# cxjyxxme/deep-online-video-stabilization

Hardware: AMD Instinct MI355X
Metric: stabilized frames/sec (720p, before_ch=31) (higher is better)
Workload: dtype f32 (bf16x3 split MFMA, f32 accumulate); 1 GPU; BASELINE.json configs[1]: v2_93 net, 1280x720, 1 stream(s)/GPU, batch=1 per stream, 13-ch stack from a 32-deep ring (lags 1,2,4,8,16,32; --before-ch 31 ignored as in the reference), ResNet-v2-50 regressor + 4x4 multi-grid warp + feedback; one independent stream set per GPU (replicas only); height=720, width=1280, streams_per_gpu=1, refine=1, operand_mode=4, launches_per_frame=64, hip_graph=True

## Files before the change

deep-online-video-stabilization_amd/csrc/conv.hip:

```cpp
#include "conv.h"
#include "prof.h"
#include <climits>
#include <cstdio>
#include <cstdlib>
#include <algorithm>
#include <string>
#include <vector>

#include "conv_kernel.h"
#include "conv_ring_kernel.h"
#include "conv_astat_kernel.h"
#include "conv_patch_kernel.h"
#include "conv_b2b_kernel.h"

template <int PAIR>
__device__ __forceinline__ void conv_splitk_reduce_body(const ConvArgs& p, const ConvPair& pr) {
    const size_t q = (size_t)blockIdx.x * 256 + threadIdx.x;
    const int c4n = p.Cout / 4;
    if (q >= (size_t)p.M * c4n) return;
    const int m = (int)(q / c4n);
    const int n = (int)(q - (size_t)m * c4n) * 4;
    const bool t1 = PAIR && m >= pr.m_tower;
    const size_t slab = (size_t)p.M * p.Cout;
    const float* src = p.partial + (size_t)m * p.Cout + n;
// ... 428 lines not shown
    return r.nbuf == 1 ? launch_one_nb<BM, BN, BK, WM, WN, MODE, 1>(a, st) : launch_one_nb<BM, BN, BK, WM, WN, MODE, 2>(a, st);
}

template <int BM, int BN, int BK, int WM, int WN>
static int launch_one(const ConvRoute& r, const ConvArgs& a, hipStream_t st) {
    if (r.mode == 2) return launch_one_t<BM, BN, BK, WM, WN, 2>(r, a, st);
    if (r.mode == 0) return launch_one_t<BM, BN, BK, WM, WN, 0>(r, a, st);
    return launch_one_t<BM, BN, BK, WM, WN, 1>(r, a, st);
}

static int launch_igemm(const ConvRoute& r, const ConvArgs& a, hipStream_t st) {
    if (r.bk == 32) {
        if (r.tile == T128x128) return launch_one<128, 128, 32, 64, 64>(r, a, st);
        if (r.tile == T128x64) return launch_one<128, 64, 32, 64, 32>(r, a, st);
        return launch_one<64, 64, 32, 32, 32>(r, a, st);
    }
    if (r.tile == T128x128) return launch_one<128, 128, 16, 64, 64>(r, a, st);
    if (r.tile == T128x64) return launch_one<128, 64, 16, 64, 32>(r, a, st);
    return launch_one<64, 64, 16, 32, 32>(r, a, st);
}

static int device_cus(int& cus) {
    static int cached = 0;
    if (cached == 0) {
        int dev = 0, n = 0;
        if (hipGetDevice(&dev) != hipSuccess || hipDeviceGetAttribute(&n, hipDeviceAttributeMultiprocessorCount, dev) != hipSuccess || n <= 0) {
            stabnet_set_error("conv: cannot read the CU count");
            return STABNET_ERR_LAUNCH;
        }
        cached = n;
    }
    cus = cached;
    return STABNET_OK;
}
static thread_local int g_last_launch_kind = -1;

template <int B>
static bool launch_ring_operand(const ConvRoute& r, const ConvArgs& a, int grid, hipStream_t st) {
    const int key = 100 * r.mode + 10 * r.kg + r.pro;
    if (key == 10) { conv_ring_f32_kernel<0, B><<<grid, 256, 0, st>>>(a); return true; }
    if (key == 110) { conv_ring_f32_kernel<1, B><<<grid, 256, 0, st>>>(a); return true; }
    if (key == 210) { conv_ring_f32_kernel<2, B><<<grid, 256, 0, st>>>(a); return true; }
    if constexpr (B != 1) {
        if (key == 11) { conv_ring_f32_kernel<0, B, 1, 1><<<grid, 256, 0, st>>>(a); return true; }
        if (key == 21) { conv_ring_f32_kernel<0, B, 2, 1><<<grid, 512, 0, st>>>(a); return true; }
    }
    if constexpr (B == 0 || B == 2 || B == 3) {
        if (key == 30) { conv_ring_f32_kernel<0, B, 3><<<grid, 768, 0, st>>>(a); return true; }
        if (key == 130) { conv_ring_f32_kernel<1, B, 3><<<grid, 768, 0, st>>>(a); return true; }
    }
    if constexpr (B == 4) {
        if (key == 20) { conv_ring_f32_kernel<0, B, 2, 0><<<grid, 512, 0, st>>>(a); return true; }
        if (key == 120) { conv_ring_f32_kernel<1, B, 2, 0><<<grid, 512, 0, st>>>(a); return true; }
    }
    return false;
}

static int launch_ring_route(const ConvRoute& r, const ConvArgs& a, hipStream_t st) {
    int cus = 0;
    if (const int rc = device_cus(cus)) return rc;
    const int grid = ring_grid(r, a, cus).gx;
    bool ok = false;
    switch (r.operand) {
        case 0: ok = launch_ring_operand<0>(r, a, grid, st); break;
        case 1: ok = launch_ring_operand<1>(r, a, grid, st); break;
        case 2: ok = launch_ring_operand<2>(r, a, grid, st); break;
        case 3: ok = launch_ring_operand<3>(r, a, grid, st); break;
        case 4: ok = launch_ring_operand<4>(r, a, grid, st); break;
        default: break;
    }
    SN_REQUIRE(ok, "conv: no conv_ring_f32_kernel<%d, %d, %d, %d>", r.mode, r.operand, r.kg, r.pro);
    SN_LAUNCH_CHECK("conv_ring_f32_kernel");
    return STABNET_OK;
}

static int launch_astat(const ConvRoute& r, const ConvArgs& a, hipStream_t st) {
    int cus = 0;
    if (const int rc = device_cus(cus)) return rc;
    const int bm = r.astat_bm;
    SN_REQUIRE(bm == 32 && a.K % 32 == 0 && (size_t)bm * a.K * 6 <= (size_t)SN_ASTAT_A_BYTES && a.splitk == 1,
               "conv: the A-stationary kernel takes BM %d x K %d without a K split only if the planes fit %d bytes", bm, a.K, SN_ASTAT_A_BYTES);
    const ConvGrid g = astat_grid(a, bm, cus);
    const dim3 grid(g.gx, g.gy);
    conv_astat_f32_kernel<32><<<grid, 256, 0, st>>>(a);
    SN_LAUNCH_CHECK("conv_astat_f32_kernel");
    return STABNET_OK;
}

template <int PH, int PW, int WR, int NS>
static int launch_patch_one(const ConvArgs& a, int cus, hipStream_t st) {
    const size_t lds = sn_patch_lds_bytes(PH, PW, a.Cin);
    auto kern = conv_patch_f32_kernel<PH, PW, WR, NS>;
    static size_t configured = 64 * 1024;
    if (lds > configured) {
        hipError_t e = hipFuncSetAttribute(reinterpret_cast<const void*>(kern), hipFuncAttributeMaxDynamicSharedMemorySize, (int)SN_PATCH_LDS_MAX);
        if (e != hipSuccess) {
            stabnet_set_error("conv: hipFuncSetAttribute(%zu B LDS) failed: %s", SN_PATCH_LDS_MAX, hipGetErrorString(e));
            return STABNET_ERR_LAUNCH;
        }
        configured = SN_PATCH_LDS_MAX;
    }
    const ConvGrid g = patch_grid(a, PH, PW, WR, cus);
    const dim3 grid(g.gx, g.gy);
    kern<<<grid, 256, lds, st>>>(a);
    SN_LAUNCH_CHECK("conv_patch_f32_kernel");
    return STABNET_OK;
}
static int launch_patch(const ConvRoute& r, const ConvArgs& a, hipStream_t st) {
    int cus = 0;
    if (const int rc = device_cus(cus)) return rc;
    SN_REQUIRE(a.KH == 3 && a.KW == 3 && a.stride == 1 && a.pad == 1 && a.up == 1 && a.Cin % 32 == 0 &&
                   (a.splitk == 1 || (a.splitk == 2 && a.steps_per_split * 2 == conv_total_steps(a))) && a.Ho == a.H && a.Wo == a.W && r.patch_cfg >= 1 &&
                   r.patch_cfg <= SN_PATCH_FORMS &&
                   sn_patch_lds_bytes(g_patch_forms[r.patch_cfg - 1].ph, g_patch_forms[r.patch_cfg - 1].pw, a.Cin) <= SN_PATCH_LDS_MAX,
               "conv: the patch-stationary kernel takes 3x3 / pad 1 / stride 1 over Cin %d (a multiple of 32) without a K split or with two equal K halves only if the planes fit %zu bytes",
               a.Cin, SN_PATCH_LDS_MAX);
    return r.patch_cfg == 1 ? launch_patch_one<8, 8, 1, 3>(a, cus, st) : launch_patch_one<8, 8, 2, 3>(a, cus, st);
}

size_t conv_weight_image_floats(int Cout, int K) { return (size_t)cdiv(Cout, 64) * (size_t)(K / 32) * 3072; }

__device__ __forceinline__ unsigned weight_split_head(float& x0, float& x1) {
    const float top = __builtin_bit_cast(float, 0x7F7F0000u), fmax = __builtin_bit_cast(float, 0x7F7FFFFFu);
    const float h0 = (fabsf(x0) > top && fabsf(x0) <= fmax) ? copysignf(top, x0) : x0;
    const float h1 = (fabsf(x1) > top && fabsf(x1) <= fmax) ? copysignf(top, x1) : x1;
    const unsigned p = sn_pack_bf16(h0, h1);
    x0 = sn_sub_f32(x0, __builtin_bit_cast(float, p << 16));
    x1 = sn_sub_f32(x1, __builtin_bit_cast(float, p & 0xffff0000u));
    return p;
}
__device__ __forceinline__ SnSplit3 weight_split3(const f32x4 x) {
    float a = x.x, b = x.y, c = x.z, d = x.w;
    typedef unsigned u32x2 __attribute__((ext_vector_type(2)));
    u32x2 h, m, l;
    h.x = weight_split_head(a, b); h.y = weight_split_head(c, d);
    m.x = sn_split_level(a, b); m.y = sn_split_level(c, d);
    l.x = sn_pack_bf16(a, b); l.y = sn_pack_bf16(c, d);
    SnSplit3 s;
    s.h = __builtin_bit_cast(sn_bf16x4, h); s.m = __builtin_bit_cast(sn_bf16x4, m); s.l = __builtin_bit_cast(sn_bf16x4, l);
    return s;
}

__device__ __forceinline__ void weight_split_image_thread(const float* __restrict__ w, int Cout, int K, uint4* __restrict__ img, long i) {
    const int steps = K / 32;
    const int lane = (int)(i & 63), j = (int)((i >> 6) & 1), wn = (int)((i >> 7) & 1);
    const long ts = i >> 8;
    const int ks = (int)(ts % steps), nt = (int)(ts / steps);
    const int n = nt * 64 + wn * 32 + (lane & 31), g = lane >> 5;
    f32x4 lo = {0.f, 0.f, 0.f, 0.f}, hi = lo;
    if (n < Cout) {
        const float* r = w + (size_t)n * K + ks * 32 + 16 * j + 4 * g;
        lo = *reinterpret_cast<const f32x4*>(r);
        hi = *reinterpret_cast<const f32x4*>(r + 8);
    }
    const SnSplit3 a = weight_split3(lo), b = weight_split3(hi);
    uint4* out = img + ts * 768 + (size_t)(wn * 6 + j) * 64 + lane;
    out[0] = __builtin_bit_cast(uint4, SN_CAT8(a.h, b.h));
    out[2 * 64] = __builtin_bit_cast(uint4, SN_CAT8(a.m, b.m));
    out[4 * 64] = __builtin_bit_cast(uint4, SN_CAT8(a.l, b.l));
}

__global__ __launch_bounds__(256) void weight_split_image_kernel(const float* __restrict__ w, int Cout, int K, uint4* __restrict__ img) {
    const long i = (long)blockIdx.x * 256 + threadIdx.x;
    if (i >= (long)((Cout + 63) / 64) * (K / 32) * 256) return;
    weight_split_image_thread(w, Cout, K, img, i);
}

// ... 129 lines not shown
                       a.M, a.Cout, a.K, a.splitk);
    if (rc) return rc;
    if (a.splitk > 1) {
        const size_t q = (size_t)a.M * (a.Cout / 4);
        const bool rec2 = prof != nullptr && prof->begin(st);
        conv_splitk_reduce_pair_kernel<<<cdiv((long)q, 256), 256, 0, st>>>(a, pr);
        if (rec2) prof->end(st, PK_KERNEL_SPLITK_REDUCE, 0.0, 4.0 * (double)a.M * a.Cout * (a.splitk + 1));
        SN_LAUNCH_CHECK("conv_splitk_reduce_pair_kernel");
    }
    return STABNET_OK;
}

bool conv_b2b_supported(const ConvArgs& c2, const ConvArgs& c3) {
    const bool g2 = c2.KH == 3 && c2.KW == 3 && c2.pad == 1 && c2.up == 1 && !c2.rowrun && (c2.stride == 1 || c2.stride == 2) &&
                    c2.Cin == c2.Cout && (c2.Cout == 64 || c2.Cout == 128) && c2.in_scale_expected == 0 && c2.in_scale == nullptr;
    const bool g3 = c3.KH == 1 && c3.KW == 1 && c3.pad == 0 && c3.stride == 1 && c3.up == 1 && !c3.rowrun && c3.Cin == c2.Cout &&
                    (c3.x_ld == 0 || c3.x_ld == c3.Cin) && c3.Cout % c2.Cout == 0 && c3.N == c2.N && c3.H == c2.Ho && c3.W == c2.Wo &&
                    c3.in_scale_expected == 0 && c3.in_scale == nullptr;
    return sw().b2b && sw().ring && g2 && g3;
}

int conv_b2b_launch(const ConvArgs& c2, const ConvArgs& c3, hipStream_t st, Prof* prof) {
    SN_REQUIRE(conv_b2b_supported(c2, c3), "conv b2b: unsupported geometry");
    SN_REQUIRE(c2.div_hw_mul != 0 && c3.div_hw_mul != 0 && c2.M == c3.M, "conv b2b: conv_plan() not called on both convolutions");
    SN_REQUIRE(c2.x && c2.w && c3.w && c3.y && c2.out_scale && c2.out_shift, "conv b2b: null pointer");
    SN_REQUIRE(c2.bias == nullptr && c2.residual == nullptr, "conv b2b: the 3x3 convolution takes no bias / residual");
    int cus = 0;
    if (const int rc = device_cus(cus)) return rc;
    B2bArgs P;
    P.c2 = c2;
    P.c3 = c3;
    P.c3.splitk = 1;
    P.c3.steps_per_split = conv_total_steps(c3);
    const int tiles_m = cdiv(c2.M, 64);
    g_last_launch_kind = PK_KERNEL_CONV_B2B + (c2.Cout == 128 ? 1 : 0);
    const bool rec = prof != nullptr && prof->begin(st);
    if (c2.Cout == 64) {
        conv_b2b_f32_kernel<2><<<std::min(tiles_m, sw().b2b_wgs_per_cu * usable_cus(cus)), 256, 0, st>>>(P);
    } else {
        conv_b2b_f32_kernel<4><<<std::min(tiles_m, usable_cus(cus)), 512, 0, st>>>(P);
    }
    if (rec) prof->end(st, PK_KERNEL_CONV_B2B + (c2.Cout == 128 ? 1 : 0),
                       2.0 * c2.M * ((double)c2.K * c2.Cout + (double)c3.K * c3.Cout),
                       4.0 * ((double)c2.N * c2.H * c2.W * c2.Cin + (double)c2.K * c2.Cout + (double)c3.K * c3.Cout +
                              (double)c3.M * c3.Cout * (c3.residual ? 2 : 1)),
                       c2.M, c3.Cout, c2.K + c3.K, 1);
    SN_LAUNCH_CHECK("conv_b2b_f32_kernel");
    return STABNET_OK;
}

static int fill_args(ConvArgs& a, const float* x, const float* w, const float* bias, const float* in_scale,
                     const float* in_shift, const float* residual, int res_H, int res_W, int res_stride, float* y,
                     int N, int H, int W, int Cin, int Cout, int KH, int KW, int stride, int pad, int relu_out) {
    SN_REQUIRE(N > 0 && H > 0 && W > 0 && Cin > 0 && Cout > 0 && KH > 0 && KW > 0 && stride > 0 && pad >= 0,
               "conv2d: bad geometry");
    SN_REQUIRE(Cin % 16 == 0, "conv2d: Cin=%d must be a multiple of 16", Cin);
    SN_REQUIRE((in_scale == nullptr) == (in_shift == nullptr), "conv2d: in_scale and in_shift go together");
    a = ConvArgs{};
    a.x = x; a.w = w; a.y = y; a.bias = bias; a.in_scale = in_scale; a.in_shift = in_shift; a.residual = residual;
    a.in_scale_expected = in_scale != nullptr ? 1 : 0;
    a.N = N; a.H = H; a.W = W; a.Cin = Cin; a.Cout = Cout; a.KH = KH; a.KW = KW; a.stride = stride; a.pad = pad;
    a.up = 1;
    a.Ho = (H + 2 * pad - KH) / stride + 1;
    a.Wo = (W + 2 * pad - KW) / stride + 1;
    SN_REQUIRE(a.Ho > 0 && a.Wo > 0, "conv2d: empty output");
    a.res_H = residual ? res_H : a.Ho;
    a.res_W = residual ? res_W : a.Wo;
    a.res_stride = residual ? res_stride : 1;
    a.relu_out = relu_out;
    SN_REQUIRE((long)N * a.Ho * a.Wo * Cout < (1L << 30) && (long)N * (H + 2 * pad) * (W + 2 * pad) * Cin < (1L << 30) &&
                   (long)Cout * KH * KW * Cin < (1L << 30), "conv2d: tensors must have < 2^30 elements");
    SN_REQUIRE(KH * KW <= 64, "conv2d: filter larger than 64 taps");
    return STABNET_OK;
}

extern "C" {

int stabnet_conv_reserve_cus(int reserved) {
    const int prev = g_reserved_cus;
    g_reserved_cus = reserved < 0 ? 0 : reserved;
    return prev;
}

void stabnet_conv_tuning_override(int tile, int splitk) {
    g_force_tile = tile < 0 ? -1 : tile;
    g_force_split = splitk;
}

void stabnet_conv_tuning_profile(int profile) { g_tuning_profile = profile == 1 ? 1 : 0; }

void stabnet_conv_tuning_table_set(int M, int Cout, int K, int KH, int ring, int splitk) {
    if (M < 0) { g_tuning_runtime.clear(); return; }
    for (size_t i = 0; i < g_tuning_runtime.size(); ++i) {
        TuneEntry& e = g_tuning_runtime[i];
        if (e.M == M && e.Cout == Cout && e.K == K && e.KH == KH && e.ring == ring) {
            if (splitk > 0) e.splitk = splitk;
            else g_tuning_runtime.erase(g_tuning_runtime.begin() + i);
            return;
        }
    }
    if (splitk > 0) g_tuning_runtime.push_back({M, Cout, K, KH, ring, splitk});
}

size_t stabnet_conv2d_workspace_bytes(int N, int H, int W, int Cin, int Cout, int KH, int KW, int stride, int pad) {
    ConvArgs a;
    if (fill_args(a, nullptr, nullptr, nullptr, nullptr, nullptr, nullptr, 0, 0, 1, nullptr, N, H, W, Cin, Cout, KH, KW,
                  stride, pad, 0))
        return 0;
    ConvArgs b = a;
    b.in_scale_expected = 1;
    return std::max(conv_plan(a), conv_plan(b));
}

int stabnet_conv2d_fwd_ex(const float* x, const float* w_ohwi, const float* bias, const float* in_scale,
                          const float* in_shift, const float* residual, int res_H, int res_W, int res_stride,
                          const float* out_scale, const float* out_shift, float* y, int N, int H, int W, int Cin,
                          int Cout, int KH, int KW, int stride, int pad, int relu_out, void* workspace,
                          size_t workspace_bytes, void* stream);

int stabnet_conv2d_fwd(const float* x, const float* w_ohwi, const float* bias, const float* in_scale,
                       const float* in_shift, const float* residual, int res_H, int res_W, int res_stride, float* y,
                       int N, int H, int W, int Cin, int Cout, int KH, int KW, int stride, int pad, int relu_out,
                       void* workspace, size_t workspace_bytes, void* stream) {
    return stabnet_conv2d_fwd_ex(x, w_ohwi, bias, in_scale, in_shift, residual, res_H, res_W, res_stride, nullptr, nullptr,
                                 y, N, H, W, Cin, Cout, KH, KW, stride, pad, relu_out, workspace, workspace_bytes, stream);
}

int stabnet_conv_last_launch_kind(void) { return g_last_launch_kind; }

int stabnet_conv2d_fwd_ex(const float* x, const float* w_ohwi, const float* bias, const float* in_scale,
                          const float* in_shift, const float* residual, int res_H, int res_W, int res_stride,
                          const float* out_scale, const float* out_shift, float* y, int N, int H, int W, int Cin,
                          int Cout, int KH, int KW, int stride, int pad, int relu_out, void* workspace,
                          size_t workspace_bytes, void* stream) {
    SN_REQUIRE(x && w_ohwi && y, "conv2d_fwd: null pointer");
    SN_REQUIRE((out_scale == nullptr) == (out_shift == nullptr), "conv2d_fwd: out_scale and out_shift go together");
    ConvArgs a;
    int rc = fill_args(a, x, w_ohwi, bias, in_scale, in_shift, residual, res_H, res_W, res_stride, y, N, H, W, Cin, Cout,
                       KH, KW, stride, pad, relu_out);
    if (rc) return rc;
    const size_t need = conv_plan(a);
    if (need > workspace_bytes || (need > 0 && workspace == nullptr)) {
        stabnet_set_error("conv2d_fwd: workspace %zu B < %zu B needed", workspace_bytes, need);
        return STABNET_ERR_WORKSPACE;
    }
    a.partial = static_cast<float*>(workspace);
    a.out_scale = out_scale;
    a.out_shift = out_shift;
    return conv_launch(a, (hipStream_t)stream);
}

int stabnet_conv2d_fwd_packed_ld(const float* x, int x_ld, const float* w_ohwi, const float* w_img, const float* bias, const float* in_scale,
                                 const float* in_shift, const float* residual, int res_H, int res_W, int res_stride,
                                 const float* out_scale, const float* out_shift, float* y, int N, int H, int W, int Cin,
                                 int Cout, int KH, int KW, int stride, int pad, int relu_out, int splitk, void* workspace,
                                 size_t workspace_bytes, void* stream);
size_t stabnet_conv_weight_image_floats(int Cout, int KH, int KW, int Cin) {
    const int K = KH * KW * Cin;
    return (Cout > 0 && K > 0 && K % 32 == 0) ? conv_weight_image_floats(Cout, K) : 0;
}

int stabnet_conv_weight_split_image(const float* w_ohwi, int Cout, int KH, int KW, int Cin, float* w_img, void* stream) {
    SN_REQUIRE(w_ohwi && w_img, "conv_weight_split_image: null pointer");
    SN_REQUIRE(Cin % 32 == 0, "conv_weight_split_image: Cin=%d must be a multiple of 32", Cin);
    return launch_weight_split_image(w_ohwi, Cout, KH * KW * Cin, w_img, (hipStream_t)stream);
}
// ... 80 lines not shown
```

deep-online-video-stabilization_amd/csrc/conv_astat_kernel.h:

```cpp
#pragma once
#include "conv_kernel.h"

constexpr int SN_ASTAT_A_BYTES = 48 * 1024;

template <int BM>
__global__ __launch_bounds__(256, 2) void conv_astat_f32_kernel(const ConvArgs p) {
    static_assert(BM == 32 || BM == 64, "one or two 32-row blocks");
    constexpr int RB = BM / 32;
    typedef unsigned u32x2 __attribute__((ext_vector_type(2)));
    __shared__ __attribute__((aligned(16))) unsigned char lds[SN_ASTAT_A_BYTES + 4 * SN_EPI_WAVE_BYTES];

    const int tid = threadIdx.x, lane = tid & 63, wave = __builtin_amdgcn_readfirstlane(tid >> 6);
    const int steps = p.K >> 5, kq = 2 * steps;
    const ConvTile tile = conv_tile_of_block(p);
    const int m0 = tile.mt * BM, grp = tile.nt;

    {
        const int r = tid >> 3, sub = tid & 7;
        const unsigned ent = (unsigned)((r + 32 * (sub & 1)) * 16 + 8 * ((sub >> 1) & 1));
#pragma unroll
        for (int rb = 0; rb < RB; ++rb) {
            const int row = min(m0 + rb * 32 + r, p.M - 1);
            const float* src = p.x + (size_t)row * p.x_ld + sub * 4;
            for (int ks0 = 0; ks0 < steps; ks0 += 4) {
                f32x4 v[4];
#pragma unroll
                for (int i = 0; i < 4; ++i) v[i] = *reinterpret_cast<const f32x4*>(src + 32 * min(ks0 + i, steps - 1));
                __builtin_amdgcn_sched_barrier(0);
#pragma unroll
                for (int i = 0; i < 4; ++i) {
                    float a = v[i].x, b = v[i].y, c = v[i].z, d = v[i].w;
                    u32x2 h, m, l;
                    h.x = sn_split_level(a, b); h.y = sn_split_level(c, d);
                    m.x = sn_split_level(a, b); m.y = sn_split_level(c, d);
                    l.x = sn_pack_bf16(a, b); l.y = sn_pack_bf16(c, d);
                    unsigned char* dst = lds + (unsigned)((rb * kq + 2 * min(ks0 + i, steps - 1) + (sub >> 2)) * 3072) + ent;
                    *reinterpret_cast<u32x2*>(dst) = h;
                    *reinterpret_cast<u32x2*>(dst + 1024) = m;
                    *reinterpret_cast<u32x2*>(dst + 2048) = l;
                }
            }
        }
    }
    __syncthreads();

    const int nblk = 2 * ((p.Cout + 63) >> 6);
    const int bpg = (((nblk + (int)gridDim.y - 1) / (int)gridDim.y) + 3) & ~3;
    const int b_end = min(min(nblk, (grp + 1) * bpg), (p.Cout + 31) >> 5);
    int b = grp * bpg + wave;
    if (b >= b_end) return;
    const unsigned scratch = (unsigned)(size_t)(__attribute__((address_space(3))) void*)lds + (unsigned)(SN_ASTAT_A_BYTES + wave * SN_EPI_WAVE_BYTES);
    const f32x4* lp = reinterpret_cast<const f32x4*>(p.w) + ((size_t)(b >> 1) * steps * 12 + (b & 1) * 6) * 64 + lane;
    const unsigned char* afrag = lds + lane * 16;
    const int items = ((b_end - b + 3) >> 2) * steps;
    int l_item = 0, l_ks = 0;
    auto load = [&](f32x4 (&dst)[6]) {
#pragma unroll
        for (int i = 0; i < 6; ++i) dst[i] = lp[i * 64];
        const int adv = l_item + 1 >= items ? 0 : (l_ks + 1 < steps ? 768 : 768 * (steps + 1));
        lp += adv;
        ++l_item;
        l_ks = l_ks + 1 < steps ? l_ks + 1 : 0;
        __builtin_amdgcn_sched_barrier(0);
    };
    f32x16 acc[RB][1];
    auto zero = [&]() {
#pragma unroll
        for (int rb = 0; rb < RB; ++rb)
#pragma unroll
            for (int e = 0; e < 16; ++e) acc[rb][0][e] = 0.f;
    };
    int ks = 0;
    auto item = [&](const f32x4 (&B)[6]) {
#pragma unroll
        for (int j = 0; j < 2; ++j) {
#pragma unroll
            for (int rb = 0; rb < RB; ++rb) {
                const unsigned char* ap = afrag + (unsigned)((rb * kq + 2 * ks + j) * 3072);
                SnPlanes A;
                A.h = *reinterpret_cast<const sn_u32x4*>(ap);
                A.m = *reinterpret_cast<const sn_u32x4*>(ap + 1024);
                A.l = *reinterpret_cast<const sn_u32x4*>(ap + 2048);
                sn_mfma_split3_pk(acc[rb][0], A, B[j], B[2 + j], B[4 + j]);
            }
        }
        if (++ks == steps) {
            conv_epilogue<RB, 1>(acc, p, m0, b * 32, lane, 0, scratch);
            b += 4;
            ks = 0;
            zero();
        }
    };
    f32x4 B0[6], B1[6], B2[6];
    zero();
    load(B0);
    load(B1);
    for (int it = 0; it < items; it += 3) {
        load(B2); item(B0);
        if (it + 1 >= items) break;
        load(B0); item(B1);
        if (it + 2 >= items) break;
        load(B1); item(B2);
    }
}
```

deep-online-video-stabilization_amd/csrc/layers.hip:

```cpp
#include "layers.h"
#include <algorithm>

__global__ __launch_bounds__(256) void pad_channels_kernel(const float* __restrict__ x, float* __restrict__ y,
                                                           long npix, int C, int Cp) {
    const long q = (long)blockIdx.x * 256 + threadIdx.x;
    const int f4 = Cp / 4;
    if (q >= npix * f4) return;
    const long pix = q / f4;
    const int c = (int)(q - pix * f4) * 4;
    const float* s = x + pix * C;
    float4 v;
    v.x = (c + 0 < C) ? s[c + 0] : 0.f;
    v.y = (c + 1 < C) ? s[c + 1] : 0.f;
    v.z = (c + 2 < C) ? s[c + 2] : 0.f;
    v.w = (c + 3 < C) ? s[c + 3] : 0.f;
    *reinterpret_cast<float4*>(y + pix * Cp + c) = v;
}

__global__ __launch_bounds__(256) void max_pool_kernel(const float* __restrict__ x, float* __restrict__ y, int N, int H,
                                                       int W, int C, int Ho, int Wo, int k, int stride, int pt, int pl,
                                                       const float* __restrict__ scale, const float* __restrict__ shift) {
    const unsigned q = sn_xcd_band(blockIdx.x, gridDim.x) * 256u + threadIdx.x;
    const unsigned c4n = (unsigned)C / 4u;
    if (q >= (unsigned)N * Ho * Wo * c4n) return;
    const int c = (int)(q % c4n) * 4;
    unsigned r = q / c4n;
    const int ox = (int)(r % (unsigned)Wo); r /= (unsigned)Wo;
    const int oy = (int)(r % (unsigned)Ho);
    const int n = (int)(r / (unsigned)Ho);
    float4 m = make_float4(-INFINITY, -INFINITY, -INFINITY, -INFINITY);
    for (int dy = 0; dy < k; ++dy) {
        const int iy = oy * stride - pt + dy;
        if (iy < 0 || iy >= H) continue;
        for (int dx = 0; dx < k; ++dx) {
            const int ix = ox * stride - pl + dx;
            if (ix < 0 || ix >= W) continue;
            const float4 v = *reinterpret_cast<const float4*>(x + (((long)n * H + iy) * W + ix) * C + c);
            m.x = v.x >= m.x ? v.x : m.x; m.y = v.y >= m.y ? v.y : m.y; m.z = v.z >= m.z ? v.z : m.z; m.w = v.w >= m.w ? v.w : m.w;
        }
    }
    if (scale != nullptr) {
        const float4 sc = *reinterpret_cast<const float4*>(scale + c), sh = *reinterpret_cast<const float4*>(shift + c);
        m.x = fmaxf(__builtin_fmaf(m.x, sc.x, sh.x), 0.f); m.y = fmaxf(__builtin_fmaf(m.y, sc.y, sh.y), 0.f);
        m.z = fmaxf(__builtin_fmaf(m.z, sc.z, sh.z), 0.f); m.w = fmaxf(__builtin_fmaf(m.w, sc.w, sh.w), 0.f);
    }
    *reinterpret_cast<float4*>(y + (((long)n * Ho + oy) * Wo + ox) * C + c) = m;
}

__global__ __launch_bounds__(256) void bn_fold_kernel(const float* __restrict__ gamma, const float* __restrict__ beta,
                                                      const float* __restrict__ mean, const float* __restrict__ var,
                                                      float eps, int G, float* __restrict__ scale,
                                                      float* __restrict__ shift) {
    const int i = blockIdx.x * 256 + threadIdx.x;
    if (i >= G) return;
    const float inv = (1.0f / sqrtf(var[i] + eps)) * gamma[i];
    scale[i] = inv;
    shift[i] = beta[i] - mean[i] * inv;
}

__global__ __launch_bounds__(256) void gap_bn_relu_partial_kernel(const float* __restrict__ x, const float* __restrict__ scale,
                                                                  const float* __restrict__ shift, int HW, int C,
                                                                  int rows_per_chunk, float* __restrict__ partial) {
    __shared__ float4 part[16][16];
    const int q = threadIdx.x & 15, rl = threadIdx.x >> 4;
    const int c = blockIdx.x * 64 + q * 4;
    const int n = blockIdx.z;
    const int r0 = blockIdx.y * rows_per_chunk, r1 = min(HW, r0 + rows_per_chunk);
    float4 s = make_float4(0.f, 0.f, 0.f, 0.f);
    if (c < C) {
        const float4 sc = *reinterpret_cast<const float4*>(scale + c), sh = *reinterpret_cast<const float4*>(shift + c);
        const float* p = x + (size_t)n * HW * C + c;
        for (int ib = r0 + rl; ib < r1; ib += 128) {
            float4 xv[8];
#pragma unroll
            for (int j = 0; j < 8; ++j) {
                const int i = ib + 16 * j;
                xv[j] = (i < r1) ? *reinterpret_cast<const float4*>(p + (size_t)i * C) : make_float4(0.f, 0.f, 0.f, 0.f);
            }
#pragma unroll
            for (int j = 0; j < 8; ++j) {
                if (ib + 16 * j < r1) {
                    const float4 v = xv[j];
                    s.x += fmaxf(__builtin_fmaf(v.x, sc.x, sh.x), 0.f); s.y += fmaxf(__builtin_fmaf(v.y, sc.y, sh.y), 0.f);
                    s.z += fmaxf(__builtin_fmaf(v.z, sc.z, sh.z), 0.f); s.w += fmaxf(__builtin_fmaf(v.w, sc.w, sh.w), 0.f);
                }
            }
        }
    }
    part[rl][q] = s;
    __syncthreads();
    if (rl == 0 && c < C) {
        float4 t = part[0][q];
        for (int i = 1; i < 16; ++i) { const float4 u = part[i][q]; t.x += u.x; t.y += u.y; t.z += u.z; t.w += u.w; }
        *reinterpret_cast<float4*>(partial + ((size_t)n * gridDim.y + blockIdx.y) * C + c) = t;
    }
}

__global__ __launch_bounds__(256) void gap_finalize_kernel(const float* __restrict__ partial, int chunks, int HW, int C,
                                                           float* __restrict__ out) {
    const int c = blockIdx.x * 256 + threadIdx.x;
    const int n = blockIdx.y;
    if (c >= C) return;
    float t = 0.f;
    for (int k = 0; k < chunks; ++k) t += partial[((size_t)n * chunks + k) * C + c];
    out[(size_t)n * C + c] = t / (float)HW;
}

template <int MR>
__global__ __launch_bounds__(256) void fc_kernel(const float* __restrict__ x, const float* __restrict__ w,
                                                 const float* __restrict__ b, float* __restrict__ y, int M, int K,
                                                 int Nout, int relu, int m_begin) {
    const int n = blockIdx.x * 4 + (threadIdx.x >> 6);
    const int lane = threadIdx.x & 63;
    if (n >= Nout) return;
    float acc[MR];
#pragma unroll
    for (int i = 0; i < MR; ++i) acc[i] = 0.f;
    const float* wr = w + (size_t)n * K;
    for (int kb = 0; kb < K; kb += 8 * 256) {
        float4 wv[8];
#pragma unroll
// ... 237 lines not shown
```

deep-online-video-stabilization_amd/csrc/net.hip:

```cpp
#include <string>
#include <vector>
#include <cstring>
#include <algorithm>
#include <mutex>
#include <unordered_map>

#include "conv.h"
#include "layers.h"
#include "prof.h"
#include "ring.h"
#include "train_layers.h"
#include "warp.h"
#include "../../include/stabnet_hip.h"

extern "C" int stabnet_black_accumulate(const float* black, int* all_black, long n, void* stream);

enum { PK_CONV_W = 0, PK_BIAS = 1, PK_GAMMA = 2, PK_BETA = 3, PK_MEAN = 4, PK_VAR = 5, PK_FC_W = 6, PK_FC_B = 7 };
enum { S_PAD = 0, S_CONV = 1, S_POOL = 2, S_GAP = 3, S_FC = 4, S_CONV_B2B = 5  };
static int fc_launches(int M) { int n = 0, m0 = 0; for (; M - m0 > 8; m0 += 16) ++n; return n + (m0 < M ? 1 : 0); }
static const long EXT_IN = -2, EXT_OUT = -3, NONE = -1;

struct ParamEntry {
    std::string name;
    int kind;
// ... 837 lines not shown
int stabnet_net_num_steps(const void* netp) { return netp ? (int)static_cast<const Net*>(netp)->steps.size() : -1; }
int stabnet_net_step_info_fields(void) { return STABNET_SI_FIELDS; }

int stabnet_net_step_info(const void* netp, int step, int cus, long* info, int cap) {
    const Net* net = static_cast<const Net*>(netp);
    SN_REQUIRE(net && info, "step_info: null pointer");
    SN_REQUIRE(!net->keep_all, "step_info: inference plans only (keep_activations = 0)");
    SN_REQUIRE(step >= 0 && step < (int)net->steps.size(), "step_info: step %d outside the plan's %d steps", step, (int)net->steps.size());
    SN_REQUIRE(cus > 0 && cap >= STABNET_SI_FIELDS, "step_info: cus %d must be positive and info hold %d fields (cap %d)", cus, STABNET_SI_FIELDS, cap);
    const Step& s = net->steps[step];
    for (int i = 0; i < STABNET_SI_FIELDS; ++i) info[i] = 0;
    info[STABNET_SI_KIND] = s.kind;
    if (s.kind != S_CONV) return STABNET_OK;
    const float* params = reinterpret_cast<const float*>((size_t)1 << 40);
    const float* fold = reinterpret_cast<const float*>((size_t)2 << 40);
    float* ws = reinterpret_cast<float*>((size_t)3 << 40);
    const float* w_img = nullptr;
    const ConvArgs a = bind_conv(net, s, params, fold, ws, w_img);
    const ConvRoute r = conv_route(a, net->bf16_operands, w_img != nullptr, true);
    const ConvGrid g = conv_grid(r, a, cus);
    info[STABNET_SI_N] = a.N; info[STABNET_SI_H] = a.H; info[STABNET_SI_W] = a.W; info[STABNET_SI_CIN] = a.Cin;
    info[STABNET_SI_HO] = a.Ho; info[STABNET_SI_WO] = a.Wo; info[STABNET_SI_COUT] = a.Cout;
    info[STABNET_SI_KH] = a.KH; info[STABNET_SI_KW] = a.KW; info[STABNET_SI_STRIDE] = a.stride; info[STABNET_SI_PAD] = a.pad;
    info[STABNET_SI_X_LD] = a.x_ld; info[STABNET_SI_RES_LD] = a.res_ld;
    info[STABNET_SI_RES_H] = a.res_H; info[STABNET_SI_RES_W] = a.res_W; info[STABNET_SI_RES_STRIDE] = a.res_stride;
    info[STABNET_SI_ROWRUN] = a.rowrun; info[STABNET_SI_RELU_OUT] = a.relu_out;
    info[STABNET_SI_M] = a.M; info[STABNET_SI_K] = a.K;
    info[STABNET_SI_IN_OFF] = s.in_off; info[STABNET_SI_IN_BASE] = s.in_base; info[STABNET_SI_IN_FLOATS] = (long)s.in_floats;
    info[STABNET_SI_OUT_OFF] = s.out_off; info[STABNET_SI_OUT_FLOATS] = (long)a.M * a.Cout;
    info[STABNET_SI_RES_OFF] = s.res_off >= 0 ? s.res_off : -1; info[STABNET_SI_RES_FLOATS] = (long)s.res_floats;
    info[STABNET_SI_SCRATCH_OFF] = (long)net->act_floats;
    info[STABNET_SI_SCRATCH_FLOATS] = r.reduce ? (long)a.splitk * a.M * a.Cout : 0;
    info[STABNET_SI_W_OFF] = s.w_off; info[STABNET_SI_BIAS_OFF] = s.b_off >= 0 ? s.b_off : -1;
    info[STABNET_SI_PRO_BN_OFF] = a.in_scale ? s.bn_off : -1;
    info[STABNET_SI_OUT_BN_OFF] = s.obn_off >= 0 ? s.obn_off : -1;
    info[STABNET_SI_MERGED_OFF] = s.fvec_off >= 0 ? (long)(2 * net->G + net->stem_w_floats) + s.fvec_off : -1;
    info[STABNET_SI_W_ROWRUN_OFF] = a.rowrun ? (long)(2 * net->G) : -1;
    info[STABNET_SI_W_IMAGE_OFF] = w_img ? (long)(w_img - fold) : -1;
    info[STABNET_SI_INF_PREACTIVATED] = s.inf_preactivated; info[STABNET_SI_PROLOGUE] = a.in_scale ? 1 : 0;
    info[STABNET_SI_SPLITK] = a.splitk; info[STABNET_SI_STEPS_PER_SPLIT] = a.steps_per_split; info[STABNET_SI_TOTAL_STEPS] = conv_plan_total_steps(a);
    info[STABNET_SI_FAMILY] = r.family; info[STABNET_SI_MODE] = r.mode; info[STABNET_SI_OPERAND] = r.operand; info[STABNET_SI_KG] = r.kg;
    info[STABNET_SI_PRO] = r.pro; info[STABNET_SI_NBUF] = r.nbuf; info[STABNET_SI_BK] = r.bk; info[STABNET_SI_TILE] = r.tile;
    info[STABNET_SI_ASTAT_BM] = r.astat_bm; info[STABNET_SI_PATCH_CFG] = r.patch_cfg; info[STABNET_SI_REDUCE] = r.reduce;
    info[STABNET_SI_PROF_KIND] = r.prof_kind;
    info[STABNET_SI_TILES] = g.tiles; info[STABNET_SI_WGS] = g.wgs; info[STABNET_SI_GX] = g.gx; info[STABNET_SI_GY] = g.gy; info[STABNET_SI_GZ] = g.gz;
    info[STABNET_SI_DIV_HW_MUL] = a.div_hw_mul; info[STABNET_SI_DIV_HW_SHIFT] = a.div_hw_shift;
    info[STABNET_SI_DIV_W_MUL] = a.div_w_mul; info[STABNET_SI_DIV_W_SHIFT] = a.div_w_shift;
    info[STABNET_SI_LDS_BYTES] = r.family == CONV_ASTAT ? (long)conv_astat_plane_bytes(r, a) : r.family == CONV_PATCH ? (long)conv_patch_lds_bytes(r, a) : 0;
    info[STABNET_SI_LDS_LIMIT] = r.family == CONV_ASTAT ? (long)conv_astat_plane_limit() : r.family == CONV_PATCH ? (long)conv_patch_lds_limit() : 0;
    return STABNET_OK;
}

int stabnet_net_run_steps(const void* netp, const float* params, const float* fold, const float* x_tensor, float* theta,
                          void* workspace, size_t workspace_bytes, int first, int last, void* stream) {
    const Net* net = static_cast<const Net*>(netp);
    SN_REQUIRE(net && params && fold && workspace, "net_run_steps: null pointer");
    SN_REQUIRE(!net->keep_all, "net_run_steps: inference plans only (keep_activations = 0)");
    SN_REQUIRE(first >= 0 && first <= last && last < (int)net->steps.size(), "net_run_steps: steps %d..%d outside the plan's %d steps", first, last,
               (int)net->steps.size());
    if (workspace_bytes < stabnet_net_workspace_bytes(netp)) {
        stabnet_set_error("net_run_steps: workspace %zu B < %zu B needed", workspace_bytes, stabnet_net_workspace_bytes(netp));
        return STABNET_ERR_WORKSPACE;
    }
    const bool fused_head = head_fused_supported(net->N, net->t_last.C, net->fc_dims);
    for (int i = first; i <= last; ++i) {
        const Step& s = net->steps[i];
        SN_REQUIRE(s.kind != S_PAD || x_tensor != nullptr, "net_run_steps: step %d reads x_tensor", i);
        SN_REQUIRE(!(s.kind == S_FC && s.out_off == EXT_OUT) || theta != nullptr, "net_run_steps: step %d writes theta", i);
    }
    SN_REQUIRE(!(fused_head && last + 1 == (int)net->steps.size()) || theta != nullptr, "net_run_steps: the last step writes theta");
    int rc = sn_check_device(params, "net_run_steps: params", (hipStream_t)stream);
    if (rc == 0) rc = sn_check_device(workspace, "net_run_steps: workspace", (hipStream_t)stream);
    if (rc) return rc;
    return run_steps(net, params, fold, x_tensor, theta, static_cast<float*>(workspace), (hipStream_t)stream, first, last);
}

int stabnet_ring_init(float* frames_ring, float* masks_ring, const float* first_frame, int S, int depth, int H, int W,
                      void* stream) {
    SN_REQUIRE(frames_ring && masks_ring && first_frame && S > 0 && S <= 65535 && depth > 0 && H > 0 && W > 0,
               "ring_init: bad arguments");
    return launch_ring_init(frames_ring, masks_ring, first_frame, S, depth, (long)H * W, (hipStream_t)stream);
}

int stabnet_deploy_frame(const void* netp, const float* params, const float* fold, float* frames_ring,
                         float* masks_ring, int depth, int* head, const int* lags, int n_lags, const float* cur_frame,
                         int refine, int grid_h, int grid_w, float do_crop_rate, float* theta, float* out_img,
                         float* black, float* x_map, float* y_map, float* Hs, float* frame_fb, int* all_black,
                         void* workspace, size_t workspace_bytes, void* stream, void* profp) {
    const Net* net = static_cast<const Net*>(netp);
    SN_REQUIRE(net && params && fold && frames_ring && masks_ring && lags && cur_frame && theta && out_img && black &&
                   x_map && y_map && Hs && frame_fb && workspace, "deploy_frame: null pointer");
    SN_REQUIRE(depth > 0 && head != nullptr && refine >= 1, "deploy_frame: bad ring arguments");
    SN_REQUIRE(2 * n_lags + 1 == net->in_ch && n_lags <= 7, "deploy_frame: %d lags do not make %d channels", n_lags,
               net->in_ch);
    SN_REQUIRE((grid_h + 1) * (grid_w + 1) * 2 == net->n_theta, "deploy_frame: grid does not match n_theta");
    if (workspace_bytes < stabnet_net_workspace_bytes(netp)) {
        stabnet_set_error("deploy_frame: workspace %zu B < %zu B needed", workspace_bytes, stabnet_net_workspace_bytes(netp));
        return STABNET_ERR_WORKSPACE;
    }
    int rc = check_warp_args(net->N, net->H, net->W, 1, grid_h, grid_w);
    if (rc) return rc;
    if ((rc = sn_check_device(params, "deploy_frame: params", (hipStream_t)stream)) != 0) return rc;
    if ((rc = sn_check_device(workspace, "deploy_frame: workspace", (hipStream_t)stream)) != 0) return rc;
    hipStream_t st = (hipStream_t)stream;
    Prof* prof = static_cast<Prof*>(profp);
    float* ws = static_cast<float*>(workspace);
    RingLags rl{};
    rl.n = n_lags;
    for (int i = 0; i < n_lags; ++i) {
        SN_REQUIRE(lags[i] > 0 && lags[i] <= depth, "deploy_frame: lag %d outside the ring", lags[i]);
        rl.lag[i] = lags[i];
    }
    const long hw = (long)net->H * net->W;
    const float* cur = cur_frame;
    float* x16 = ws + net->steps[0].out_off;
    const bool fused_push = (refine == 1);
    for (int j = 0; j < refine; ++j) {
        bool rec = prof && prof->begin(st);
        if (net->stem_rowrun)
            rc = launch_stack_assemble_bordered(frames_ring, masks_ring, cur, net->N, depth, head, rl, net->H, net->W, 3, x16, st);
        else
            rc = launch_stack_assemble(frames_ring, masks_ring, cur, net->N, depth, head, rl, hw, net->in_ch_act, x16, st);
        if (rec) prof->end(st, PK_KERNEL_ASSEMBLE, 0, 4.0 * net->N * hw * (net->in_ch + net->in_ch_act));
        if (rc) return rc;
        MeshTail mt{grid_h, grid_w, 1.0f / do_crop_rate, Hs, fused_push ? head : nullptr, depth, false};
        mt.prefetch_src = cur;
        rc = run_forward(net, params, fold, nullptr, theta, ws, st, prof, true, &mt);
        if (rc) return rc;
        if (!mt.done) {
            rec = prof && prof->begin(st);
            rc = launch_mesh(theta, 1, net->N, grid_h, grid_w, 1.0f / do_crop_rate, nullptr, Hs, st, nullptr, mt.head_adv, depth);
            if (rec) prof->end(st, PK_KERNEL_MESH, 0, 4.0 * net->N * (net->n_theta + grid_h * grid_w * 9));
            if (rc) return rc;
        }
        if (fused_push) {
            WarpPush wp{frames_ring, masks_ring, frame_fb, all_black, head, depth};
            rec = prof && prof->begin(st);
            rc = launch_sample_push(Hs, cur, net->N, net->H, net->W, grid_h, grid_w, out_img, black, x_map, y_map, wp, st);
            if (rec) prof->end(st, PK_KERNEL_WARP, 0, net->N * (32.0 * hw + 776.0) + (all_black ? 8.0 * net->N * hw : 0.0));
            return rc;
        }
        rec = prof && prof->begin(st);
        rc = launch_sample(Hs, cur, net->N, net->H, net->W, 1, grid_h, grid_w, out_img, black, x_map, y_map, st);
        if (rec) prof->end(st, PK_KERNEL_WARP, 0, net->N * (20.0 * hw + 776.0));
        if (rc) return rc;
        if (all_black != nullptr && (rc = stabnet_black_accumulate(black, all_black, (long)net->N * hw, stream)) != 0) return rc;
        const bool last = (j == refine - 1);
        rec = prof && prof->begin(st);
        if (last)
            rc = launch_ring_push(frames_ring, masks_ring, net->N, depth, head, out_img, black, hw, frame_fb, st);
        else
            rc = launch_ring_push(frame_fb, nullptr, net->N, 1, nullptr, out_img, black, hw, nullptr, st);
        if (rec) prof->end(st, PK_KERNEL_PUSH, 0, 4.0 * net->N * hw * 4);
        if (rc) return rc;
        if (!last) cur = frame_fb;
    }
    return launch_ring_advance(head, depth, st);
}

}

struct TrainLayout {
    size_t bn_scale, bn_shift, bn_mean, bn_invstd, GA, GB, T1, T2, T3, fcg0, fcg1, partial, fcpart, coef, wt, wt_img, fw_img, argmax, splitk, slabs, total;
    size_t fcx[4];
    size_t fcpart_floats;
    size_t splitk_bytes, slab_floats;
// ... 477 lines not shown
```

include/stabnet_hip.h:

```cpp
#ifndef STABNET_HIP_H
#define STABNET_HIP_H

#include <stddef.h>
#include <stdint.h>

#ifdef __cplusplus
extern "C" {
#endif

const char* stabnet_last_error(void);
int stabnet_abi_version(void);


int stabnet_get_4_pts(const float* theta, int N, int grid_h, int grid_w, float do_crop_rate,
                      float* pts1, float* pts2, float* Hs, void* stream);

int stabnet_transformer_fwd(const float* pts2, const float* U, int N, int H, int W, int C, int grid_h, int grid_w,
                            float* out, float* black, float* x_map, float* y_map, float* Hs, void* stream);

int stabnet_warp_fwd(const float* theta, const float* U, int N, int H, int W, int C, int grid_h, int grid_w,
                     float do_crop_rate, float* out, float* black, float* x_map, float* y_map, float* Hs,
                     float* pts2, void* stream);

int stabnet_maps_from_hs_fwd(const float* Hs, const float* U, int N, int H, int W, int C, int grid_h, int grid_w,
// ... 30 lines not shown
                                 size_t workspace_bytes, void* stream);
int stabnet_conv2d_packed_kind(int N, int H, int W, int Cin, int Cout, int KH, int KW, int stride, int pad, int prologue, int splitk);
int stabnet_conv_last_launch_kind(void);
int stabnet_conv3x3_conv1x1_fwd(const float* x, int x_ld, const float* w2_ohwi, const float* mid_scale, const float* mid_shift,
                                const float* w3_ohwi, const float* bias3, const float* residual, int res_H, int res_W,
                                int res_stride, int res_ld, const float* out_scale, const float* out_shift, float* y, int N, int H,
                                int W, int C, int Cout, int stride, int relu_out, void* stream);

int stabnet_net_create(void** net, int N, int H, int W, int in_ch, int n_theta, int keep_activations);
void stabnet_net_destroy(void* net);
int stabnet_net_set_bf16_operands(void* net, int on);
int stabnet_net_num_params(const void* net);
int stabnet_net_param_info(const void* net, int idx, char* name, int name_cap, long* offset, int* kind, int* dims4,
                           int* aux);
size_t stabnet_net_param_floats(const void* net);
size_t stabnet_net_trainable_floats(const void* net);
size_t stabnet_net_bn_channels(const void* net);
size_t stabnet_net_workspace_bytes(const void* net);
double stabnet_net_flops(const void* net);
int stabnet_net_num_launches(const void* net);
int stabnet_deploy_frame_launches(const void* net, int grid_h, int grid_w);
int stabnet_net_activation_info(const void* net, const char* name, long* offset, int* dims4);

int stabnet_net_fold_bn(const void* net, const float* params, float* fold, float eps, void* stream);
size_t stabnet_net_fold_floats(const void* net);

int stabnet_backbone_fwd_infer(const void* net, const float* params, const float* fold, const float* x_tensor,
                               float* theta, void* workspace, size_t workspace_bytes, void* stream, void* prof);

enum {
    STABNET_SI_KIND = 0,
    STABNET_SI_N, STABNET_SI_H, STABNET_SI_W, STABNET_SI_CIN, STABNET_SI_HO, STABNET_SI_WO, STABNET_SI_COUT, STABNET_SI_KH, STABNET_SI_KW,
    STABNET_SI_STRIDE, STABNET_SI_PAD, STABNET_SI_X_LD, STABNET_SI_RES_LD, STABNET_SI_RES_H, STABNET_SI_RES_W, STABNET_SI_RES_STRIDE,
    STABNET_SI_ROWRUN, STABNET_SI_RELU_OUT, STABNET_SI_M, STABNET_SI_K,
    STABNET_SI_IN_OFF, STABNET_SI_IN_BASE, STABNET_SI_IN_FLOATS, STABNET_SI_OUT_OFF, STABNET_SI_OUT_FLOATS, STABNET_SI_RES_OFF,
    STABNET_SI_RES_FLOATS, STABNET_SI_SCRATCH_OFF, STABNET_SI_SCRATCH_FLOATS,
    STABNET_SI_W_OFF, STABNET_SI_BIAS_OFF, STABNET_SI_PRO_BN_OFF, STABNET_SI_OUT_BN_OFF, STABNET_SI_MERGED_OFF, STABNET_SI_W_ROWRUN_OFF,
    STABNET_SI_W_IMAGE_OFF, STABNET_SI_INF_PREACTIVATED, STABNET_SI_PROLOGUE,
    STABNET_SI_SPLITK, STABNET_SI_STEPS_PER_SPLIT, STABNET_SI_TOTAL_STEPS,
    STABNET_SI_FAMILY, STABNET_SI_MODE, STABNET_SI_OPERAND, STABNET_SI_KG, STABNET_SI_PRO, STABNET_SI_NBUF, STABNET_SI_BK, STABNET_SI_TILE,
    STABNET_SI_ASTAT_BM, STABNET_SI_PATCH_CFG, STABNET_SI_REDUCE, STABNET_SI_PROF_KIND,
    STABNET_SI_TILES, STABNET_SI_WGS, STABNET_SI_GX, STABNET_SI_GY, STABNET_SI_GZ,
    STABNET_SI_DIV_HW_MUL, STABNET_SI_DIV_HW_SHIFT, STABNET_SI_DIV_W_MUL, STABNET_SI_DIV_W_SHIFT,
    STABNET_SI_LDS_BYTES, STABNET_SI_LDS_LIMIT,
    STABNET_SI_FIELDS
};
int stabnet_net_num_steps(const void* net);
int stabnet_net_step_info_fields(void);
int stabnet_net_step_info(const void* net, int step, int cus, long* info, int cap);
int stabnet_net_run_steps(const void* net, const float* params, const float* fold, const float* x_tensor, float* theta,
                          void* workspace, size_t workspace_bytes, int first, int last, void* stream);


int stabnet_pad_channels(const float* x, float* y, long npix, int C, int Cp, void* stream);

int stabnet_stem_repack(const float* w, float* out, int Cout, int KH, int KW, int CinPad, int Cin, void* stream);

int stabnet_merge_vectors(const float* b_sc, const float* scale1, const float* shift1, int depth, int dbn, float* out, void* stream);

int stabnet_bn_fold(const float* gamma, const float* beta, const float* mean, const float* var, float eps, int G, float* scale,
                    float* shift, void* stream);

int stabnet_max_pool_fwd(const float* x, float* y, int N, int H, int W, int C, int Ho, int Wo, int k, int stride, int pt, int pl,
                         const float* scale, const float* shift, void* stream);

size_t stabnet_gap_partial_floats(int N, int HW, int C);
int stabnet_gap_bn_relu(const float* x, const float* scale, const float* shift, int N, int HW, int C, float* out, float* partial,
                        size_t partial_floats, void* stream);

int stabnet_fc_fwd(const float* x, const float* w, const float* b, float* y, int M, int K, int Nout, int relu, void* stream);

int stabnet_head_fused_supported(int N, int C, const int* fc_dims);
size_t stabnet_head_gap_partial_floats(int N, int HW, int C);
int stabnet_head_gap_fc1(const float* x, const float* scale, const float* shift, int N, int HW, int C, float* partial,
                         size_t partial_floats, float* gap_out, const float* w, const float* b, float* y, int Nout, void* stream);
int stabnet_head_theta_mesh(const float* x, const float* w, const float* b, int N, int K, int n_theta, float* theta, int grid_h,
                            int grid_w, float do_crop_rate, float* Hs, int* head_adv, int depth, const float* prefetch_src, int pf_H,
                            int pf_W, void* stream);


int stabnet_ring_init(float* frames_ring, float* masks_ring, const float* first_frame, int S, int depth, int H, int W,
                      void* stream);

int stabnet_deploy_frame(const void* net, const float* params, const float* fold, float* frames_ring,
                         float* masks_ring, int depth, int* head, const int* lags, int n_lags, const float* cur_frame,
                         int refine, int grid_h, int grid_w, float do_crop_rate, float* theta, float* out_img,
                         float* black, float* x_map, float* y_map, float* Hs, float* frame_fb, int* all_black,
                         void* workspace, size_t workspace_bytes, void* stream, void* prof);

int stabnet_prof_create(void** prof, int max_records);
void stabnet_prof_destroy(void* prof);
int stabnet_prof_reset(void* prof);
int stabnet_prof_record_empty(void* prof, void* stream);
int stabnet_prof_num_records(const void* prof);
int stabnet_prof_record(const void* prof, int idx, int* kind, float* ms, double* flops, double* bytes);
int stabnet_prof_record_shape(const void* prof, int idx, int* shape4);
const char* stabnet_prof_kind_name(int kind);

int stabnet_probe_mfma_f32(float* out , int blocks, int iters,
                           unsigned long long* stamps ,
                           void* stream);
double stabnet_probe_mfma_f32_flops(int blocks, int iters);
int stabnet_probe_hbm_copy(const float* src, float* dst, long n_floats, void* stream);
int stabnet_probe_comm_proxy(const float* src, float* dst, long n_floats, int workgroups, int lds_bytes, unsigned long long* stamps,
                             void* stream);
int stabnet_conv_reserve_cus(int reserved);


int stabnet_transformer_bwd(const float* pts2, const float* Hs, const float* U, const float* x_map, const float* y_map,
                            const float* d_out, const float* d_xmap, const float* d_ymap, const float* dmap_scale, int N,
                            int H, int W, int C, int grid_h, int grid_w, float* d_pts2, void* workspace, void* stream);

int stabnet_interp_bwd(const float* x, const float* y, const float* d_out, int N, int H, int W, int C, float* d_im,
                       int accumulate, void* workspace, void* stream);

int stabnet_slice_channel(const float* x, long npix, int C, int c, float* out, void* stream);
int stabnet_interleave2(const float* a, const float* b, long n, float* out, void* stream);

int stabnet_axpb(const float* x, float a, float b, long n, float* y, void* stream);

size_t stabnet_masked_mse_workspace_bytes(int N);
int stabnet_masked_mse_sums(const float* a, const float* b, const float* black, const float* m2, int N, long hw,
                            float* sums, void* workspace, void* stream);
int stabnet_masked_mse_grad(const float* a, const float* b, const float* black, const float* m2, const float* sums,
                            float coef, int N, long hw, float* ga, int accumulate_a, float* gb, void* stream);

int stabnet_feature_loss(const float* matches, const float* mask, const float* x_map, const float* y_map, int N, int H,
                         int W, int max_matches, float gcoef, float* value, float* d_xmap, float* d_ymap, float* dscale,
                         float* warped, void* stream);

int stabnet_mesh_losses(const float* theta, const float* d_pts2_warp, int N, int grid_h, int grid_w, float do_crop_rate,
                        float id_mul, float w_id, float w_dist, float w_cons, float use_black, float w_black,
                        float* losses4, float* d_theta, void* stream);


size_t stabnet_conv2d_wgrad_workspace_bytes(int N, int H, int W, int Cin, int Cout, int KH, int KW, int stride, int pad);
int stabnet_conv2d_wgrad(const float* x, const float* dy, float* dw, const float* in_scale, const float* in_shift,
                         int N, int H, int W, int Cin, int Cout, int KH, int KW, int stride, int pad, void* workspace,
                         size_t workspace_bytes, void* stream);

size_t stabnet_conv2d_wgrad_bias_workspace_bytes(int N, int H, int W, int Cin, int Cout);
int stabnet_conv2d_wgrad_bias(const float* x, const float* dy, float* dw, float* d_bias, const float* in_scale, const float* in_shift,
                              int N, int H, int W, int Cin, int Cout, void* workspace, size_t workspace_bytes, void* stream);

size_t stabnet_conv2d_wgrad_rowrun_workspace_bytes(int N, int H, int W, int Cin, int Cout, int KH, int KW, int stride, int pad);
int stabnet_conv2d_wgrad_rowrun(const float* x, const float* dy, float* dw, int N, int H, int W, int Cin, int CinPad, int Cout,
                                int KH, int KW, int stride, int pad, void* workspace, size_t workspace_bytes, void* stream);

size_t stabnet_conv2d_dgrad_workspace_bytes(int N, int H, int W, int Cin, int Cout, int KH, int KW, int stride, int pad);
int stabnet_conv2d_dgrad(const float* dy, const float* w_ohwi, float* dx, const float* residual, int N, int H, int W,
                         int Cin, int Cout, int KH, int KW, int stride, int pad, void* workspace,
                         size_t workspace_bytes, void* stream);

size_t stabnet_conv2d_wgrad_layers_workspace_bytes(int L, int T, const int* geom, const long* bias_off);
int stabnet_conv2d_wgrad_layers(int L, int T, const int* geom, const float* const* tensors, float* grads, size_t grads_floats,
                                const long* dw_off, const long* bias_off, void* workspace, size_t workspace_bytes, void* stream);

int stabnet_pack_dgrad_weights_table(const float* params, size_t params_floats, float* wt, size_t wt_floats, int L, const long* w_off,
                                     const int* dims, void* stream);

int stabnet_conv_weight_split_images_table(const float* w_base, size_t w_floats, float* img_base, size_t img_floats, int L,
                                           const long* w_off, const long* img_off, const int* dims, void* stream);

size_t stabnet_conv2d_dgrad_split_workspace_bytes(int N, int H, int W, int Cin, int Cout, int KH, int KW, int stride, int pad);
int stabnet_conv2d_dgrad_split(const float* dy, const float* w_ohwi, float* dx, const float* residual, int N, int H, int W, int Cin,
                               int Cout, int KH, int KW, int stride, int pad, void* workspace, size_t workspace_bytes,
                               int* packed_route, void* stream);

size_t stabnet_net_train_workspace_bytes(const void* net);

int stabnet_tower_fwd_train(const void* net, float* params, const float* x_tensor, float* theta, void* workspace,
                            size_t workspace_bytes, float bn_eps, float bn_decay, void* stream, void* prof);

int stabnet_towers_fwd_train(const void* net, float* params, const float* x1, const float* x2, float* theta1, float* theta2,
                             void* workspace1, void* workspace2, size_t workspace_bytes, float bn_eps, float bn_decay,
                             void* stream, void* prof);

int stabnet_tower_bwd(const void* net, const float* params, const float* d_theta, float* grads, void* workspace,
                      size_t workspace_bytes, void* stream, void* prof);
int stabnet_tower_bwd_stage(const void* net, const float* params, const float* d_theta, float* grads, void* workspace,
                            size_t workspace_bytes, int stage, void* stream, void* prof);
int stabnet_towers_bwd_stage(const void* net, const float* params, const float* d_theta1, const float* d_theta2, float* grads,
                             void* workspace1, void* workspace2, size_t workspace_bytes, int stage, void* stream, void* prof);
int stabnet_net_num_grad_stages(void);
int stabnet_net_grad_bucket(const void* net, int stage, long* lo, long* hi);
int stabnet_net_bn_grad_range(const void* net, long* lo, long* hi);

int stabnet_net_train_bn_offsets(const void* net, long* scale_off, long* shift_off, long* mean_off, long* invstd_off);

// ... 189 lines not shown
```

Before: 663.1 frames/s.

## Size A-stationary LDS dynamically, unroll 3x3 maxpool loads, add bordered stack API

The A-stationary conv kernel now takes dynamic shared memory sized to its actual K instead of a fixed 48KB array. For small K this can let more workgroups stay resident per CU. A new query returns how many of these workgroups fit per CU. The maxpool kernel gains a fully unrolled 3x3 path that issues all nine clamped loads up front and masks out-of-bounds taps, which raises memory-level parallelism. A bordered stack-assembly entry point is also exposed.

After: 664.0 frames/s, median of 6. No clear change (+0.1%).

```diff
diff --git a/deep-online-video-stabilization_amd/csrc/conv.hip b/deep-online-video-stabilization_amd/csrc/conv.hip
--- a/deep-online-video-stabilization_amd/csrc/conv.hip
+++ b/deep-online-video-stabilization_amd/csrc/conv.hip
@@ -534,7 +534,7 @@
                "conv: the A-stationary kernel takes BM %d x K %d without a K split only if the planes fit %d bytes", bm, a.K, SN_ASTAT_A_BYTES);
     const ConvGrid g = astat_grid(a, bm, cus);
     const dim3 grid(g.gx, g.gy);
-    conv_astat_f32_kernel<32><<<grid, 256, 0, st>>>(a);
+    conv_astat_f32_kernel<32><<<grid, 256, sn_astat_lds_bytes(32, a.K), st>>>(a);
     SN_LAUNCH_CHECK("conv_astat_f32_kernel");
     return STABNET_OK;
 }
@@ -830,6 +830,13 @@
     return prev;
 }
 
+int stabnet_conv_astat_resident_wgs(int K) {
+    if (K < 32 || K % 32 != 0 || (size_t)32 * K * 6 > (size_t)SN_ASTAT_A_BYTES) return -1;
+    int n = 0;
+    if (hipOccupancyMaxActiveBlocksPerMultiprocessor(&n, conv_astat_f32_kernel<32>, 256, sn_astat_lds_bytes(32, K)) != hipSuccess) return -1;
+    return n;
+}
+
 void stabnet_conv_tuning_override(int tile, int splitk) {
     g_force_tile = tile < 0 ? -1 : tile;
     g_force_split = splitk;
diff --git a/deep-online-video-stabilization_amd/csrc/conv_astat_kernel.h b/deep-online-video-stabilization_amd/csrc/conv_astat_kernel.h
--- a/deep-online-video-stabilization_amd/csrc/conv_astat_kernel.h
+++ b/deep-online-video-stabilization_amd/csrc/conv_astat_kernel.h
@@ -2,13 +2,14 @@
 #include "conv_kernel.h"
 
 constexpr int SN_ASTAT_A_BYTES = 48 * 1024;
+constexpr size_t sn_astat_lds_bytes(int bm, int K) { return (size_t)bm * K * 6 + 4 * SN_EPI_WAVE_BYTES; }
 
 template <int BM>
 __global__ __launch_bounds__(256, 2) void conv_astat_f32_kernel(const ConvArgs p) {
     static_assert(BM == 32 || BM == 64, "one or two 32-row blocks");
     constexpr int RB = BM / 32;
     typedef unsigned u32x2 __attribute__((ext_vector_type(2)));
-    __shared__ __attribute__((aligned(16))) unsigned char lds[SN_ASTAT_A_BYTES + 4 * SN_EPI_WAVE_BYTES];
+    extern __shared__ __attribute__((aligned(16))) unsigned char lds[];
 
     const int tid = threadIdx.x, lane = tid & 63, wave = __builtin_amdgcn_readfirstlane(tid >> 6);
     const int steps = p.K >> 5, kq = 2 * steps;
@@ -49,7 +50,7 @@
     const int b_end = min(min(nblk, (grp + 1) * bpg), (p.Cout + 31) >> 5);
     int b = grp * bpg + wave;
     if (b >= b_end) return;
-    const unsigned scratch = (unsigned)(size_t)(__attribute__((address_space(3))) void*)lds + (unsigned)(SN_ASTAT_A_BYTES + wave * SN_EPI_WAVE_BYTES);
+    const unsigned scratch = (unsigned)(size_t)(__attribute__((address_space(3))) void*)lds + (unsigned)(BM * p.K * 6 + wave * SN_EPI_WAVE_BYTES);
     const f32x4* lp = reinterpret_cast<const f32x4*>(p.w) + ((size_t)(b >> 1) * steps * 12 + (b & 1) * 6) * 64 + lane;
     const unsigned char* afrag = lds + lane * 16;
     const int items = ((b_end - b + 3) >> 2) * steps;
diff --git a/deep-online-video-stabilization_amd/csrc/layers.hip b/deep-online-video-stabilization_amd/csrc/layers.hip
--- a/deep-online-video-stabilization_amd/csrc/layers.hip
+++ b/deep-online-video-stabilization_amd/csrc/layers.hip
@@ -29,14 +29,35 @@
     const int oy = (int)(r % (unsigned)Ho);
     const int n = (int)(r / (unsigned)Ho);
     float4 m = make_float4(-INFINITY, -INFINITY, -INFINITY, -INFINITY);
-    for (int dy = 0; dy < k; ++dy) {
-        const int iy = oy * stride - pt + dy;
-        if (iy < 0 || iy >= H) continue;
-        for (int dx = 0; dx < k; ++dx) {
-            const int ix = ox * stride - pl + dx;
-            if (ix < 0 || ix >= W) continue;
-            const float4 v = *reinterpret_cast<const float4*>(x + (((long)n * H + iy) * W + ix) * C + c);
-            m.x = v.x >= m.x ? v.x : m.x; m.y = v.y >= m.y ? v.y : m.y; m.z = v.z >= m.z ? v.z : m.z; m.w = v.w >= m.w ? v.w : m.w;
+    if (k <= 3) {
+        float4 v[9];
+        bool in[9];
+#pragma unroll
+        for (int dy = 0; dy < 3; ++dy) {
+#pragma unroll
+            for (int dx = 0; dx < 3; ++dx) {
+                const int iy = oy * stride - pt + dy, ix = ox * stride - pl + dx;
+                in[dy * 3 + dx] = dy < k && dx < k && iy >= 0 && iy < H && ix >= 0 && ix < W;
+                const int cy = min(max(iy, 0), H - 1), cx = min(max(ix, 0), W - 1);
+                v[dy * 3 + dx] = *reinterpret_cast<const float4*>(x + (((long)n * H + cy) * W + cx) * C + c);
+            }
+        }
+        __builtin_amdgcn_sched_barrier(0);
+#pragma unroll
+        for (int t = 0; t < 9; ++t) {
+            m.x = (in[t] && v[t].x >= m.x) ? v[t].x : m.x; m.y = (in[t] && v[t].y >= m.y) ? v[t].y : m.y;
+            m.z = (in[t] && v[t].z >= m.z) ? v[t].z : m.z; m.w = (in[t] && v[t].w >= m.w) ? v[t].w : m.w;
+        }
+    } else {
+        for (int dy = 0; dy < k; ++dy) {
+            const int iy = oy * stride - pt + dy;
+            if (iy < 0 || iy >= H) continue;
+            for (int dx = 0; dx < k; ++dx) {
+                const int ix = ox * stride - pl + dx;
+                if (ix < 0 || ix >= W) continue;
+                const float4 v = *reinterpret_cast<const float4*>(x + (((long)n * H + iy) * W + ix) * C + c);
+                m.x = v.x >= m.x ? v.x : m.x; m.y = v.y >= m.y ? v.y : m.y; m.z = v.z >= m.z ? v.z : m.z; m.w = v.w >= m.w ? v.w : m.w;
+            }
         }
     }
     if (scale != nullptr) {
diff --git a/deep-online-video-stabilization_amd/csrc/net.hip b/deep-online-video-stabilization_amd/csrc/net.hip
--- a/deep-online-video-stabilization_amd/csrc/net.hip
+++ b/deep-online-video-stabilization_amd/csrc/net.hip
@@ -943,6 +943,16 @@
     return launch_ring_init(frames_ring, masks_ring, first_frame, S, depth, (long)H * W, (hipStream_t)stream);
 }
 
+int stabnet_stack_assemble_bordered(const float* frames_ring, const float* masks_ring, const float* cur_frame, int S, int depth,
+                                    const int* head, const int* lags, int n_lags, int H, int W, int border, float* out, void* stream) {
+    SN_REQUIRE(frames_ring && masks_ring && cur_frame && head && lags && out && S > 0 && S <= 65535 && depth > 0 && H > 0 && W > 0 &&
+               n_lags >= 1 && n_lags <= 7 && border >= 0, "stack_assemble_bordered: bad arguments");
+    RingLags rl{};
+    rl.n = n_lags;
+    for (int l = 0; l < n_lags; ++l) rl.lag[l] = lags[l];
+    return launch_stack_assemble_bordered(frames_ring, masks_ring, cur_frame, S, depth, head, rl, H, W, border, out, (hipStream_t)stream);
+}
+
 int stabnet_deploy_frame(const void* netp, const float* params, const float* fold, float* frames_ring,
                          float* masks_ring, int depth, int* head, const int* lags, int n_lags, const float* cur_frame,
                          int refine, int grid_h, int grid_w, float do_crop_rate, float* theta, float* out_img,
diff --git a/include/stabnet_hip.h b/include/stabnet_hip.h
--- a/include/stabnet_hip.h
+++ b/include/stabnet_hip.h
@@ -136,6 +136,9 @@
 int stabnet_ring_init(float* frames_ring, float* masks_ring, const float* first_frame, int S, int depth, int H, int W,
                       void* stream);
 
+int stabnet_stack_assemble_bordered(const float* frames_ring, const float* masks_ring, const float* cur_frame, int S, int depth,
+                                    const int* head, const int* lags, int n_lags, int H, int W, int border, float* out, void* stream);
+
 int stabnet_deploy_frame(const void* net, const float* params, const float* fold, float* frames_ring,
                          float* masks_ring, int depth, int* head, const int* lags, int n_lags, const float* cur_frame,
                          int refine, int grid_h, int grid_w, float do_crop_rate, float* theta, float* out_img,
@@ -159,6 +162,8 @@
 int stabnet_probe_comm_proxy(const float* src, float* dst, long n_floats, int workgroups, int lds_bytes, unsigned long long* stamps,
                              void* stream);
 int stabnet_conv_reserve_cus(int reserved);
+
+int stabnet_conv_astat_resident_wgs(int K);
 
 
 int stabnet_transformer_bwd(const float* pts2, const float* Hs, const float* U, const float* x_map, const float* y_map,
```
